# Prayforhanluo/HiCHap_master

Measured on AMD Instinct MI355X. Metric: ICE iterations/sec on 10 kb whole-genome matrix (also nnz*iters/sec), higher is better.
Workload: dtype f64; 1 GPU; hg19-10kb-diploid-wholegenome; n_bins=607282, nnz_upper=4998527599, resolution_bp=10000, parallelism=single GPU, entries_stored=9997055198, slots_u32=160483740, slots_u16=3332512024, payload_bytes=14837255808, tiles=88993, units=88985, hbm_bytes_matrix=15785038153

## Files before the change

### hichap_master_amd/_lib.py

```python
from __future__ import annotations

import ctypes as C
import os

_HERE = os.path.dirname(os.path.abspath(__file__))
LIB_PATH = os.environ.get("HH_LIB") or os.path.join(_HERE, "libhichap_hip.so")

HH_OK = 0


class HipLibraryError(RuntimeError):

    def __init__(self, code, msg):
        super().__init__(f"[hh rc={code}] {msg}")
        self.code = code


class MatrixInfo(C.Structure):
    _fields_ = [(n, C.c_int64) for n in (
        "n_bins", "row_lo", "row_hi", "nnz_upper", "n_entries", "n_slots", "n_tiles",
        "n_units", "n_wide", "device_bytes", "n_slots_narrow", "payload_bytes")] + [
        (n, C.c_int32) for n in ("n_chroms", "ignore_diags", "cis_only", "device", "band_w", "n_units_flat")] + [
        ("n_band", C.c_int64), ("payload_bytes_flat", C.c_int64)] + [
        (n, C.c_int32) for n in ("band_w4", "upper")]
# ... 47 lines not shown
    "hh_ice_n_groups": (C.c_int, [P, PI32]),
    "hh_ice_marg_local": (C.c_int, [P, I32, P, P]),
    "hh_ice_set_marg": (C.c_int, [P, P, I32, I64, P, P]),
    "hh_ice_filter_nnz": (C.c_int, [P, P]),
    "hh_ice_filter_count_mad": (C.c_int, [P, P]),
    "hh_ice_update": (C.c_int, [P, P]),
    "hh_ice_active_groups": (C.c_int, [P, PI32, P]),
    "hh_ice_iterations_done": (C.c_int, [P, PI32]),
    "hh_ice_run": (C.c_int, [P, I32, P]),
    "hh_ice_finalize": (C.c_int, [P, P, P, P, P, P, P]),
    "hh_ice_last_sweep_timing": (C.c_int, [P, PF64, PI32, PF64]),
    "hh_ice_swept_bytes": (C.c_int, [P, PI64]),
    "hh_ice_get_bias": (C.c_int, [P, P, P]),
    "hh_ice_set_bias": (C.c_int, [P, P, P]),
    "hh_ice_uband_fallbacks": (C.c_int, [P, PI64, P]),
    "hh_sweep_trace": (C.c_int, [P, I64, PI64]),
    "hh_matrix_stream_probe": (C.c_int, [P, I32, PF64, I32]),
    "hh_comm_unique_id": (C.c_int, [P]),
    "hh_comm_init": (C.c_int, [P, I32, I32, C.POINTER(P)]),
    "hh_comm_free": (C.c_int, [P]),
    "hh_comm_allgather": (C.c_int, [P, I64, P, P, P]),
    "hh_comm_reduce_scatter": (C.c_int, [P, I64, P, P, P]),
    "hh_ice_set_column_exchange": (C.c_int, [P, I32, I32, P, P, P, P, P]),
    "hh_ice_balance_sharded": (C.c_int, [P, C.POINTER(IceOpts), I32, I32, P, P, P, P, P, P, P, P, PF64, P]),
    "hh_ice_balance_cis_local": (C.c_int, [P, C.POINTER(IceOpts), I32, I64, P, P, P, P, P, P, P, PF64, P]),
    "hh_ice_filters_sharded": (C.c_int, [P, I32, P, P, P, P]),
    "hh_ice_run_sharded": (C.c_int, [P, I32, P, P, P, I32, P]),
    "hh_dense_rowstats": (C.c_int, [P, I32, I64, P, P, P, P, I32, P]),
    "hh_dense_symvc": (C.c_int, [P, I32, I64, P, P, F64, F64, P, I32, P]),
    "hh_twostep": (C.c_int, [P, P, P, I64, P, P, P, P, I32, P]),
# ... 143 lines not shown
```

### hichap_master_amd/csrc/build.hip

```cpp
#include <algorithm>
#include <cmath>
#include <numeric>

#include <chrono>
#include <cstdio>

#include "ice_internal.hpp"

namespace hh {

struct PxErr {
    unsigned long long first;
    int code;
};

constexpr int kOccCopies = 64;

template <class Id, class Cnt>
__global__ __launch_bounds__(256) void k_px_check(const Id* __restrict__ b1, const Id* __restrict__ b2,
                                                  const Cnt* __restrict__ cnt, long long nnz, long long n_bins,
                                                  const int32_t* __restrict__ chrom_of, int ignore_diags,
                                                  int cis_only, int32_t* __restrict__ A, int32_t* __restrict__ B,
                                                  uint32_t* __restrict__ kc, unsigned* __restrict__ occ,
                                                  unsigned* __restrict__ big, int occ_max,
// ... 115 lines not shown
    if (q >= n) return;
    const long long i = (long long)(keys[q] & imask);
    keys[q] = (unsigned long long)(uint32_t)A[i] | ((unsigned long long)kc[i] << 32);
}

struct PxRows {
    const int32_t* A;
    const int32_t* B;
    const uint32_t* kc;
    const long long* up_ptr;
    const unsigned long long* lkeys;
    const long long* lo_ptr;
    long long row_lo, nloc;
    int nJ, band_w, band_w4;
    int upper;
    uint16_t* cnt;
    uint16_t* cntn;
    int32_t* row_band;
    long long* row_wide;
    long long* row_upper;
    long long* row_ent;
    double* diag;
    double* row_nnz2;
    double* row_sum2;
    const int32_t* tile_of;
    const long long* tile_ent;
    const uint32_t* tile_rp;
    const long long* tile_entn;
    const uint32_t* tile_rpn;
    uint32_t* pay;
// ... 2 lines not shown
    uint32_t* band4;
    const long long* wide_ptr;
    int32_t* wide_col;
    double* wide_cnt;
};

template <int PASS>
__global__ __launch_bounds__(256) void k_px_rows(PxRows p) {
    const long long w = ((long long)blockIdx.x * blockDim.x + threadIdx.x) >> 6;
    if (w >= p.nloc) return;
    const int lane = threadIdx.x & 63;
    const long long r = p.row_lo + w;
    const long long rb = w / kR;
    const int k = (int)(w % kR);
    const unsigned long long lt = (1ull << lane) - 1ull;
    int curJ = -1;
    long long tw = 0, tn = 0, pos = 0, posn = 0;
    long long nb_lane = 0, sum_lane = 0, ent_wave = 0, wide_wave = 0, upper_wave = 0;
    long long wpos = PASS == 1 ? p.wide_ptr[w] : 0;
    double dg = 0.0;
    auto flush = [&]() {
        if (curJ < 0) return;
        if (PASS == 0) {
            if (lane == 0) {
                p.cnt[w * p.nJ + curJ] = (uint16_t)tw;
                p.cntn[w * p.nJ + curJ] = (uint16_t)tn;
            }
        } else {
            const long long pw = (tw + 3) & ~3LL, pn = (tn + 7) & ~7LL;
            for (long long q = tw + lane; q < pw; q += 64) p.pay[pos - tw + q] = 0u;
            for (long long q = tn + lane; q < pn; q += 64) p.payn[posn - tn + q] = 0u;
        }
    };
    auto chunk = [&](long long col, uint32_t v, bool valid) {
        if (valid && col == r) {
            dg = (double)v;
            valid = false;
        }
        if (valid) sum_lane += v;
        const long long dj = col - r;
        const bool inband = valid && p.band_w > 0 && v <= kBandMaxCnt && dj >= -p.band_w && dj <= p.band_w;
        const bool innib = valid && !inband && in_band4(dj, v, p.band_w, p.band_w4);
        if (inband || innib) {
            if (PASS == 1) {
                if (inband) {
                    p.band[w * band_stride(p.band_w) + band_slot(dj, p.band_w)] = (uint8_t)v;
                } else {
                    const long long nib = w * 2 * band4_stride(p.band_w, p.band_w4) + band4_nibble(dj, p.band_w, p.band_w4);
                    atomicOr(p.band4 + (nib >> 3), v << (4 * (nib & 7)));
                }
            }
            nb_lane += 1;
            valid = false;
        }
        const bool wide = valid && v > kCntMax;
        const unsigned long long mwl = __ballot(wide);
        if (mwl) {
// ... 220 lines not shown
    DBuf<int32_t> rband(std::max<int64_t>(nloc, 1));
    DBuf<long long> rwide(nloc + 1), rupper(std::max<int64_t>(nloc, 1)), rent(std::max<int64_t>(nloc, 1));
    PxRows P{};
    P.A = dA.p;
    P.B = dB.p;
    P.kc = dkc.p;
    P.up_ptr = up_ptr.p;
    P.lkeys = keys.p;
    P.lo_ptr = lo_ptr.p;
    P.row_lo = row_lo;
    P.nloc = nloc;
    P.nJ = nJ;
    P.band_w = W;
    P.band_w4 = W4;
    P.upper = upper_tiles_on(nJ) ? 1 : 0;
    P.cnt = cnt_w.p;
    P.cntn = cnt_n.p;
    P.row_band = rband.p;
    P.row_wide = rwide.p;
    P.row_upper = rupper.p;
    P.row_ent = rent.p;
    P.diag = m->diag.p;
    P.row_nnz2 = m->row_nnz2.p;
    P.row_sum2 = m->row_sum2.p;
    const dim3 rgrid((unsigned)((nloc * 64 + 255) / 256));
    if (nloc) hipLaunchKernelGGL((k_px_rows<0>), rgrid, dim3(256), 0, s, P);
    HIP_CHECK(hipGetLastError());
    phase("pass 0");
    std::vector<uint16_t> hc((size_t)nloc * nJ), hnarrow((size_t)nloc * nJ);
    std::vector<int32_t> hb(nloc);
// ... 98 lines not shown
```

### hichap_master_amd/csrc/ice.hip

```cpp
#include <algorithm>
#include <chrono>
#include <functional>
#include <cmath>
#include <limits>

#include "ice_internal.hpp"

namespace hh {
constexpr int kThreads = 256;

constexpr int kSweepThreads = 512;
constexpr int kSweepWaves = kSweepThreads / 64;
constexpr int kFlatU = 8;
static_assert(kFlatU == kFlatIlvU, "k_sweep_flatw walks the interleaved layout's runs");

__device__ __forceinline__ double lds_b(const double* bl, uint32_t byteoff) {
    return *reinterpret_cast<const double*>(reinterpret_cast<const char*>(bl) + byteoff);
}

__device__ __forceinline__ void tile_dot(const uint4 v, const double* __restrict__ bl, double& a0, double& a1) {
    const uint32_t w[4] = {v.x, v.y, v.z, v.w};
    double x[4];
#pragma unroll
    for (int i = 0; i < 4; ++i) x[i] = lds_b(bl, w[i] & 0xFFFFu);
// ... 1508 lines not shown
    int bytes;
    int nc, ch, bits;
};
struct UbSegs {
    UbSeg s[2];
    int n;
    uint8_t ord[kMaxUbChunks];
};
struct UbArgs {
    long long row_lo, row_hi, halo_lo, nloc, g_lo;
    const uint8_t* act;
    const uint16_t* row_group;
    const double* b;
    double* upart;
    unsigned long long* fallbacks;
};

template <int BITS>
struct UbT;
template <>
struct UbT<8> {
    typedef uint4 V;
    static constexpr int LB = 16;
    static __device__ __forceinline__ V zero() { return make_uint4(0u, 0u, 0u, 0u); }
    static __device__ __forceinline__ V ld(const uint8_t* p) { return ld16(reinterpret_cast<const uint4*>(p)); }
    template <int M>
    static __device__ __forceinline__ V shift(const V prev, const V own) {
        if (M == 0) return own;
        constexpr int B = 128 - 8 * M;
        return band_shift_q<B / 32>(prev, own, B % 32);
    }
// ... 199 lines not shown
            }
        }
        if (lane == 1) {
#pragma unroll
            for (int k = 0; k < 16; ++k) heads[16 * g + k] = FAST ? col[k] * kUbDown : col[k];
        }
#pragma unroll
        for (int k = 0; k < 16; ++k) col[k] = dpp_shl1_d(col[k]);
    }
    if (FAST) {
#pragma unroll
        for (int k = 0; k < 16; ++k) col[k] *= kUbDown;
    }
}

__device__ __forceinline__ void ub_group(const UbSegs& S, long long grp, int chunk, const UbArgs& a, long long n_bins,
                                         int fast, double* __restrict__ cbuf, double* __restrict__ cwin,
                                         double* __restrict__ rowb) {
    int si = 0;
    while (si + 1 < S.n && chunk >= S.s[si + 1].ch) ++si;
    const UbSeg& P = S.s[si];
    const int kc = chunk - P.ch;
    const long long R0 = grp * kUbGroupRows;
    const int wave = __builtin_amdgcn_readfirstlane(threadIdx.x >> 6), lane = threadIdx.x & 63;
    const long long base = P.dlo + (long long)kc * kUbChunk;
    for (int j = threadIdx.x; j < kUbCols - kUbGroupRows; j += kUbThreads) cbuf[kUbGroupRows + j] = 0.0;
    if (threadIdx.x < 16) cwin[kUbWinZero + threadIdx.x] = 0.0;
    const double up = fast ? kUbUp : 1.0;
    int bad = 0;
    for (int j = threadIdx.x; j < kUbCols; j += kUbThreads) {
        const double v = ub_bias(a.b, R0 + base + j, n_bins);
        bad |= !ub_in_range(v);
        cwin[ub_pad(j)] = v * up;
// ... 6 lines not shown
    if (fast) {
        fast = __builtin_amdgcn_readfirstlane(!__syncthreads_or(bad));
        if (!fast) {
            if (threadIdx.x == 0) atomicAdd(a.fallbacks, 1ull);
            for (int j = threadIdx.x; j < kUbCols; j += kUbThreads) cwin[ub_pad(j)] = ub_bias(a.b, R0 + base + j, n_bins);
            for (int j = threadIdx.x; j < kUbGroupRows; j += kUbThreads) rowb[j] = ub_bias(a.b, R0 + j, n_bins);
            __syncthreads();
        }
    } else {
        __syncthreads();
    }
    const long long r0 = R0 + (long long)kUbRows * wave;
    const bool rows_here = r0 < a.row_hi && r0 + kUbRows > a.row_lo;
    const bool cols_here = r0 + base < a.row_hi && r0 + kUbRows + base + kUbChunk > a.row_lo;
    const bool stored = r0 + kUbRows > a.halo_lo && r0 < a.row_hi;
    double col[16];
    double* heads = cbuf + (size_t)kUbRows * wave;
    if ((rows_here || cols_here) && stored) {
        if (P.bits == 8) {
            if (fast)
                ub_walk<8, true>(P, kc, chunk, r0, a, n_bins, heads, col, cwin, rowb);
            else
                ub_walk<8, false>(P, kc, chunk, r0, a, n_bins, heads, col, cwin, rowb);
        } else {
            if (fast)
                ub_walk<4, true>(P, kc, chunk, r0, a, n_bins, heads, col, cwin, rowb);
            else
                ub_walk<4, false>(P, kc, chunk, r0, a, n_bins, heads, col, cwin, rowb);
        }
    } else {
        for (int j = lane; j < kUbRows; j += 64) heads[j] = 0.0;
#pragma unroll
        for (int k = 0; k < 16; ++k) col[k] = 0.0;
// ... 7 lines not shown
        }
    }
    __syncthreads();
    double* __restrict__ base_p = a.upart + (size_t)(kUbArrs * chunk + 1) * a.nloc;
    for (int j = threadIdx.x; j < kUbCols; j += kUbThreads) {
        const long long c = R0 + base + j;
        if (c >= a.row_lo && c < a.row_hi) base_p[(size_t)(j / kUbGroupRows) * a.nloc + (c - a.row_lo)] = cbuf[j];
    }
}

__global__ __launch_bounds__(kUbThreads, 3) __attribute__((amdgpu_num_vgpr(68))) void k_sweep_ubands(UbSegs S, UbArgs a, long long n_bins, int xcd,
                                                                int fast) {
    __shared__ double cbuf[kUbCols];
    __shared__ double cwin[kUbWin];
    __shared__ double rowb[kUbGroupRows];
    long long grp = blockIdx.x;
    int y = blockIdx.y;
    if (xcd) {
        const long long nb = (long long)gridDim.x * gridDim.y, b = blockIdx.x + (long long)blockIdx.y * gridDim.x;
        const long long L = xcd_remap(b, nb);
        y = (int)(L % gridDim.y);
        grp = L / gridDim.y;
    }
    ub_group(S, a.g_lo + grp, S.ord[y], a, n_bins, fast, cbuf, cwin, rowb);
}

__global__ void k_ub_halo(const uint8_t* __restrict__ band, const uint8_t* __restrict__ band4, long long W8,
                          long long W4, long long row_lo, long long row_hi, long long halo_lo,
                          uint8_t* __restrict__ h8, uint8_t* __restrict__ h4) {
    const long long nh = row_lo - halo_lo;
    const long long st8 = band_stride(W8), st4 = band4_stride(W8, W4), sg = band4_seg(W8, W4);
    const long long per = W8 + (W4 > W8 ? sg : 0);
    const long long i = (long long)blockIdx.x * blockDim.x + threadIdx.x;
    if (i >= nh * per) return;
    const long long hr = i / per, j = i % per, c = halo_lo + hr;
    if (j < W8) {
        const long long d = j + 1, r = c + d;
        if (r >= row_lo && r < row_hi) h8[hr * st8 + W8 + d] = band[(r - row_lo) * st8 + (W8 - d)];
    } else {
// ... 481 lines not shown
struct hh_ice {
    hh_matrix* m = nullptr;
    hh_ice_opts o{};
    int64_t n = 0, nloc = 0;
    int32_t G = 1;
    std::vector<int64_t> glo, ghi;
    int32_t n_tiles = 0;
    DBuf<int32_t> tile_lo, tile_hi, tile_group, group_tile_ptr, blk_tile_ptr;
    DBuf<double> bias, marg, part, tile_cnt, tile_sum, tile_sq, g_cnt, g_sum;
    DBuf<unsigned> counter;
    bool stats_fresh = false;
    DBuf<double> bpart;
    int32_t nch = 0;
    int32_t nchu = 0;
    DBuf<double> upart;
    DBuf<unsigned long long> ub_fallbacks;
    DBuf<uint8_t> halo8, halo4;
    int64_t halo_lo = 0, ub_glo = 0, ub_ghi = 0;
    DBuf<uint8_t> active;
    DBuf<double> g_var, g_mean;
    DBuf<int32_t> g_iters;
    DBuf<uint8_t> g_empty;
    DBuf<long long> rank_rows;
    std::vector<int64_t> h_rank_rows;
    DBuf<unsigned long long> colpart, colacc, bmax, bfix;
    DBuf<double> fix;
    double rmax = 1.0;
    bool rmax_global = false;
    int32_t cx_world = 1, cx_rank = 0;
    int64_t cx_maxlen = 0;
// ... 36 lines not shown
static int g_flatw_waves = 11;
static int g_flatw_waves_up = 8;
static int g_flatw_pipe = 3;
static int g_sweep_ablate = 0;
static int g_tiled_pf = 1;
static int g_band_concurrent = 1;
static int g_split_tiles = 1;
static int g_conc_order = 1;
static int64_t g_conc_min_bytes = 8LL << 30;
static int64_t g_conc_ub_min_bytes = 1LL << 30;
static int g_band_rows = 0;
static int g_band_fused = 1;
static int g_band_lpt = 1;
static int g_uband = 1;
static int64_t g_uband_min_bytes = 128LL << 20;
static int g_ub_xcd = 1;
static int g_ub_fast = 1;
static int g_sweep_single = -1;
static int g_iter_events = 1;
static int64_t g_single_max_bytes = 1LL << 30;
static unsigned long long* g_trace = nullptr;
static int64_t g_trace_cap = 0, g_trace_n = 0;

template <int NB, int ABL, bool UP>
static void launch_sweep_up(const hh_matrix* m, const TileDev& T, const uint8_t* act, const double* b, double* part,
                            hipStream_t s, hipStream_t s_tiled, int which) {
    const int n_tiled = (int)(m->n_units - m->n_units_flat), n_flat = (int)m->n_units_flat;
    auto tiled = [&] {
        if (!n_tiled) return;
        HH_KTIME("k_sweep_tiled", s_tiled);
// ... 123 lines not shown
        const long long sg = band4_seg(W8, W4);
        add(m->band4.p + sg, S->halo4.p ? S->halo4.p + sg : nullptr, band4_stride(W8, W4), W8 + 1, sg, W4 - W8, 4);
    }
    HH_REQUIRE(ch <= kMaxUbChunks, "too many upper-band chunks");
    std::vector<std::pair<long long, int>> w;
    for (int k = 0; k < u.n; ++k)
        for (int c = 0; c < u.s[k].nc; ++c) {
            const long long slots = u.s[k].bits == 8 ? W8 + 1 : W4 - W8;
            w.push_back({-std::min<long long>(kUbChunk, slots + 15 - (long long)c * kUbChunk), u.s[k].ch + c});
        }
    std::stable_sort(w.begin(), w.end(), [](const auto& a, const auto& b) { return a.first < b.first; });
    for (int y = 0; y < ch; ++y) u.ord[y] = (uint8_t)w[y].second;
    return ch;
}

static UbArgs ub_args(hh_ice* S) {
    const hh_matrix* m = S->m;
    return UbArgs{m->row_lo, m->row_hi, S->halo_lo, S->nloc, S->ub_glo, S->act(), m->row_group.p, S->bias.p,
                  S->upart.p, S->ub_fallbacks.p};
}

static UbMarg ub_marg(const hh_ice* S) {
    UbMarg u{};
    u.part = S->upart.p;
    u.n = S->nchu;
    if (!S->nchu) return u;
    UbSegs segs;
    ub_segs(S, segs);
    for (int k = 0; k < segs.n; ++k)
        for (int c = 0; c < segs.s[k].nc; ++c) u.base[segs.s[k].ch + c] = segs.s[k].dlo + (long long)c * kUbChunk;
    return u;
}

static void sweep_uband(hh_ice* S, hipStream_t s) {
    UbSegs segs;
    const int ch = ub_segs(S, segs);
    const long long ng = S->ub_ghi - S->ub_glo;
    if (!ch || ng <= 0) return;
    HH_KTIME("k_sweep_ubands", s);
    hipLaunchKernelGGL(k_sweep_ubands, dim3((unsigned)ng, (unsigned)ch), dim3(kUbThreads), 0, s, segs, ub_args(S),
                       (long long)S->m->n_bins, g_ub_xcd, g_ub_fast);
    HIP_CHECK(hipGetLastError());
}

static void sweep_band(hh_ice* S, hipStream_t s) {
    if (S->nchu) {
        if (S->nloc) sweep_uband(S, s);
        return;
    }
    const hh_matrix* m = S->m;
    if (!S->nch || !S->nloc) return;
    BandSegs segs;
    const int ch = band_segs(m, segs);
    const int rows = g_band_rows ? g_band_rows : (((S->nloc + 255) / 256) * ch < 1024 ? 64 : 256);
    const bool abl = g_sweep_ablate == 1;
// ... 284 lines not shown
        } else if (k == "parse_ablate") {
            HH_REQUIRE(value >= 0 && value <= 3, "parse_ablate in [0, 3]");
            g_parse_ablate = (int)value;
        } else if (k == "flatw_waves") {
            HH_REQUIRE(value == 8 || value == 10 || value == 11, "flatw_waves: 8, 10 or 11");
            g_flatw_waves = (int)value;
        } else if (k == "flat_group") {
            HH_REQUIRE(value >= 0 && value <= 256, "flat_group: 0 (auto) .. 256");
            g_flat_group = value;
        } else if (k == "uband") {
            HH_REQUIRE(value >= 0 && value <= 2, "uband: 0 (off), 1 (auto) or 2 (always)");
            g_uband = (int)value;
        } else if (k == "ub_xcd") {
            HH_REQUIRE(value == 0 || value == 1, "ub_xcd: 0 or 1");
            g_ub_xcd = (int)value;
        } else if (k == "ub_fast") {
            HH_REQUIRE(value == 0 || value == 1, "ub_fast: 0 or 1");
            g_ub_fast = (int)value;
        } else if (k == "uband_min_bytes") {
            HH_REQUIRE(value >= 0, "uband_min_bytes >= 0");
            g_uband_min_bytes = value;
        } else if (k == "band_w") {
            HH_REQUIRE(value >= -1 && value <= kBandMaxW && (value <= 0 || value % 16 == 0),
                       "band_w: -1 (auto), 0 (off) or a multiple of 16 <= 16384");
            g_band_w = value;
        } else if (k == "conc_min_bytes") {
            HH_REQUIRE(value >= 0, "conc_min_bytes >= 0");
            g_conc_min_bytes = value;
        } else if (k == "syrk_split") {
            HH_REQUIRE(value >= -1 && value <= 64, "syrk_split in [-1, 64]");
// ... 178 lines not shown
                    S->halo8.alloc((size_t)(nh * band_stride(W8)));
                    S->halo8.zero(s);
                }
                if (W4 > W8) {
                    S->halo4.alloc((size_t)(nh * band4_stride(W8, W4)));
                    S->halo4.zero(s);
                }
                const long long nthr = nh * per;
                hipLaunchKernelGGL(k_ub_halo, dim3((unsigned)((nthr + 255) / 256)), dim3(256), 0, s, m->band.p,
                                   m->band4.p, W8, W4, (long long)m->row_lo, (long long)m->row_hi, S->halo_lo,
                                   S->halo8.p, S->halo4.p);
                HIP_CHECK(hipGetLastError());
            }
            UbSegs segs;
            S->nchu = ub_segs(S.get(), segs);
            S->upart.alloc(std::max<int64_t>((int64_t)kUbArrs * S->nchu * S->nloc, 1));
            S->upart.zero(s);
            S->ub_fallbacks.alloc(1);
            S->ub_fallbacks.zero(s);
            S->nch = 0;
        }
        S->bpart.alloc(std::max<int64_t>((int64_t)S->nch * S->nloc, 1));
        if (m->upper && m->n_cslots > 0) {
            S->colpart.alloc((size_t)m->n_cslots * kW);
            S->colpart.zero(s);
        }
        if (m->upper) {
            S->colacc.alloc((size_t)std::max<int64_t>(S->n, 1));
            S->colacc.zero(s);
            const unsigned long long one[2] = {0x3FF0000000000000ull, 0ull};
// ... 239 lines not shown
}

int hh_ice_uband_fallbacks(const hh_ice* S, int64_t* count, void* stream) {
    return guard([&] {
        HH_REQUIRE(S && count, "null");
        unsigned long long c = 0;
        if (S->nchu) {
            hipStream_t s = as_stream(stream);
            S->ub_fallbacks.download(&c, 1, s);
            HIP_CHECK(hipStreamSynchronize(s));
        }
        *count = (int64_t)c;
    });
}

int hh_ice_swept_bytes(const hh_ice* S, int64_t* bytes) {
    return guard([&] {
        HH_REQUIRE(S && bytes, "null");
        const hh_matrix* m = S->m;
        int64_t b = 4 * m->n_slots + 2 * m->n_slots_narrow + (int64_t)8 * (kR + 1) * m->n_tiles;
        if (S->nchu) {
            const long long W8 = m->band_w, W4 = m->band_w4;
            const long long per = (W8 > 0 ? W8 + 16 : 0) + (W4 > W8 ? band4_seg(W8, W4) : 0);
            b += (int64_t)per * (S->nloc + (m->row_lo - S->halo_lo));
        } else {
            b += (int64_t)m->band.n + (int64_t)m->band4.n;
        }
        *bytes = b;
    });
}

int hh_matrix_stream_probe(const hh_matrix* m, int32_t reps, double* out, int32_t nout) {
    return guard([&] {
        HH_REQUIRE(m && out && nout >= 20 && reps > 0, "stream probe: 20 outputs");
        for (int i = 0; i < nout; ++i) out[i] = 0.0;
        HIP_CHECK(hipSetDevice(m->device));
        hipStream_t s;
        HIP_CHECK(hipStreamCreateWithFlags(&s, hipStreamNonBlocking));
        hipEvent_t e0, e1;
// ... 219 lines not shown
```

### hichap_master_amd/csrc/ice_internal.hpp

```cpp
#pragma once

#include "hh_common.hpp"

namespace hh {

constexpr int kR = 512;
#ifndef HH_KWBITS
#define HH_KWBITS 13
#endif
constexpr int kWBits = HH_KWBITS;
constexpr bool kUpperBuild = HH_KWBITS <= 12;
constexpr int kW = 1 << kWBits;
constexpr uint32_t kColMask = kW - 1;
constexpr uint32_t kCntMax = 65535u;
extern int64_t g_unit_lpt;
extern int64_t g_unit_lpt_lists;
extern int64_t g_tile_cost;
extern int64_t g_unit_entries;
constexpr int64_t kMaxBins = (int64_t)1 << 30;

constexpr uint32_t kNarrowMax = 7;

constexpr int kBandChunk = 2048;
constexpr int kBandMaxW = 16384;
constexpr uint32_t kBandMaxCnt = 255u;
constexpr double kBandDensity = 0.5;
extern int64_t g_band_w;
constexpr uint32_t kBand4MaxCnt = 15u;
extern double g_band4_density;
extern double g_band8_big;
extern int64_t g_band4;
extern int64_t g_upper_tiles;
struct BandWidths {
    int32_t w8 = 0, w4 = 0;
};
BandWidths choose_band_widths(const std::vector<double>& occ, const std::vector<double>& big, int ignore_diags);
__host__ __device__ __forceinline__ int64_t band4_seg(int64_t w8, int64_t w4) { return w4 > w8 ? (w4 - w8) / 2 + 16 : 0; }
__host__ __device__ __forceinline__ int64_t band4_stride(int64_t w8, int64_t w4) { return 2 * band4_seg(w8, w4); }
__host__ __device__ __forceinline__ int64_t band4_nibble(int64_t d, int64_t w8, int64_t w4) {
    return d < 0 ? d + w4 : 2 * band4_seg(w8, w4) + (d - w8 - 1);
}
__host__ __device__ __forceinline__ bool in_band4(int64_t d, uint32_t v, int64_t w8, int64_t w4) {
    const int64_t a = d < 0 ? -d : d;
    return v > 0 && v <= kBand4MaxCnt && a > w8 && a <= w4;
}
__host__ __device__ __forceinline__ int64_t band_slot(int64_t d, int64_t W) { return d + W; }
// ... 122 lines not shown

struct hh_matrix {
    int device = 0;
    int64_t n_bins = 0, row_lo = 0, row_hi = 0;
    int32_t n_chroms = 0, ignore_diags = 1, cis_only = 0;
    std::vector<int64_t> chrom_offsets;
    int64_t nnz_upper = 0;
    int64_t n_entries = 0;
    int64_t n_tiles = 0, n_units = 0, n_part = 0, n_wide = 0, nJ = 0, nrb = 0;
    int64_t n_units_flat = 0;
    int64_t payload_bytes_flat = 0;
    int64_t n_slots = 0;
    int64_t n_slots_narrow = 0;
    int32_t band_w = 0;
    int32_t band_w4 = 0;
    int64_t n_band = 0;
    hh::DBuf<uint8_t> band;
    hh::DBuf<uint8_t> band4;
    hh::DBuf<uint32_t> pay;
    hh::DBuf<uint16_t> payn;
    hh::DBuf<int32_t> tile_J, tile_rb;
    hh::DBuf<long long> tile_ent, tile_entn;
    hh::DBuf<uint32_t> tile_rp, tile_rpn;
    hh::DBuf<int32_t> u_tlo, u_thi, u_rb, u_rlo, u_rhi, u_slot, blk_unit_ptr, blk_tile_ptr, u_order;
    hh::DBuf<uint16_t> u_glo, u_ghi, tile_perm, tile_band;
    hh::DBuf<uint32_t> tile_fw;
    hh::DBuf<int32_t> tile_frec;
    hh::DBuf<uint16_t> frec;
    hh::DBuf<uint8_t> u_whole;
    hh::DBuf<int32_t> fg_ptr, fg_unit;
// ... 69 lines not shown
```

### hichap_master_amd/csrc/matrix.hip

```cpp
#include <algorithm>
#include <atomic>
#include <chrono>
#include <cstdio>
#include <cmath>
#include <numeric>
#include <exception>
#include <mutex>
#include <thread>

#include "ice_internal.hpp"

namespace hh {

static thread_local std::string g_last_error;
int64_t g_unit_entries = 0;
int g_flat_defer = 1;
int64_t g_unit_lpt = 1;
int64_t g_unit_lpt_lists = 1;
int64_t g_flat_group = 0;
int64_t g_flat_cols = -1;
bool flat_cols_on(int32_t nJ) { return g_flat_cols > 0 || (g_flat_cols < 0 && nJ >= 32); }
int64_t g_tile_cost = 32768;
int64_t g_band_w = -1;
int64_t g_flat_max = 64;
int64_t g_build_debug = 0;
int64_t g_host_build = 0;

int64_t g_upper_tiles = -1;
bool upper_tiles_on(int32_t nJ) {
    return kUpperBuild && (g_upper_tiles > 0 || (g_upper_tiles < 0 && flat_cols_on(nJ)));
}
int64_t g_band4 = 1;
double g_band4_density = 0.25;
double g_band8_big = 0.05;

int32_t choose_band_w(const std::vector<double>& occ, int ignore_diags) {
    if (g_band_w >= 0) return (int32_t)std::min<int64_t>(g_band_w, kBandMaxW) & ~15;
    int64_t d = std::max(1, ignore_diags);
    if (d > 1) return 0;
    while (d < (int64_t)occ.size() && occ[d] >= kBandDensity) ++d;
    return (int32_t)((d - 1) & ~15LL);
}

BandWidths choose_band_widths(const std::vector<double>& occ, const std::vector<double>& big, int ignore_diags) {
    BandWidths bw;
    bw.w8 = bw.w4 = choose_band_w(occ, ignore_diags);
    if (g_band_w >= 0 || !g_band4 || std::max(1, ignore_diags) > 1) return bw;
// ... 653 lines not shown
            for (int64_t i = 0; i < nnz; ++i) {
                int64_t a, b;
                uint32_t c;
                if (!keep(i, a, b, c) || a == b || b - a > kBandMaxW + 1) continue;
                occ[b - a] += 1.0;
                if (c > kBand4MaxCnt) big[b - a] += 1.0;
            }
            for (int64_t d = 1; d < (int64_t)occ.size(); ++d) {
                big[d] = occ[d] > 0 ? big[d] / occ[d] : 0.0;
                occ[d] = d < n_bins ? occ[d] / (double)(n_bins - d) : 0.0;
            }
            const BandWidths bw = choose_band_widths(occ, big, ignore_diags);
            W = bw.w8;
            W4 = bw.w4;
        }
        auto in_band = [&](int64_t r_glob, int64_t col, uint32_t v) {
            const int64_t d = col - r_glob;
            return W > 0 && v <= kBandMaxCnt && d != 0 && d >= -W && d <= W;
        };
        auto in_nib = [&](int64_t r_glob, int64_t col, uint32_t v) { return in_band4(col - r_glob, v, W, W4); };
        std::vector<int32_t> cols(deg[nloc]);
        std::vector<uint32_t> vals(deg[nloc]);
        {
            std::vector<int64_t> pos(deg.begin(), deg.end() - 1);
            for (int64_t i = 0; i < nnz; ++i) {
                int64_t a, b;
                uint32_t c;
                if (!keep(i, a, b, c) || a == b) continue;
                if (a >= row_lo && a < row_hi) { cols[pos[a - row_lo]] = (int32_t)b; vals[pos[a - row_lo]++] = c; }
                if (b >= row_lo && b < row_hi) { cols[pos[b - row_lo]] = (int32_t)a; vals[pos[b - row_lo]++] = c; }
            }
        }
        std::vector<std::pair<int32_t, uint32_t>> tmp;
        for (int64_t r = 0; r < nloc; ++r) {
            const int64_t lo = deg[r], hi = deg[r + 1];
// ... 218 lines not shown
```

### hichap_master_amd/csrc/synth.hip

```cpp
#include <cmath>
#include <numeric>

#include "ice_internal.hpp"

namespace hh {

struct SynthDev {
    long long n;
    int n_chroms;
    int nJ;
    const int* chrom_lo;
    const float* vis;
    const signed char* sgn;
    const short* chrom;
    float A, decay, comp, trans;
    int ignore_diags, cis_only;
    unsigned long long seed;
    int band_w;
    int band_w4;
    int ordered;
    int upper;
};

__global__ void k_synth_bins(SynthDev p, float vis_sigma, float gap_frac, int comp_block,
                             float* vis, signed char* sgn) {
    const long long i = (long long)blockIdx.x * blockDim.x + threadIdx.x;
    if (i >= p.n) return;
    const int c = p.chrom[i];
    const long long local = i - p.chrom_lo[c];
    const uint64_t h = mix64(p.seed ^ mix64(0xB1A5ull + (uint64_t)i));
    const float u1 = fmaxf(u01(h), 1e-7f), u2 = u01(mix64(h));
    const float z = sqrtf(-2.f * logf(u1)) * cosf(6.2831853f * u2);
    const bool gap = u01(mix64(h ^ 0x5151ull)) < gap_frac;
    vis[i] = gap ? 0.f : expf(vis_sigma * z);
    const uint64_t hb = mix64(p.seed ^ mix64(0xC0FFEEull + ((uint64_t)c << 32) + (uint64_t)(local / comp_block)));
    sgn[i] = (hb & 1) ? 1 : -1;
// ... 53 lines not shown
    uint16_t* payn;
    uint8_t* band;
    uint32_t* band4;
    int32_t* row_band;
};

template <int PASS>
__global__ __launch_bounds__(256) void k_synth_rows(SynthDev p, long long row_lo, long long nrows, SynthOut o) {
    const long long w = ((long long)blockIdx.x * blockDim.x + threadIdx.x) >> 6;
    if (w >= nrows) return;
    const int lane = threadIdx.x & 63;
    const long long r = row_lo + w;
    const int c = p.chrom[r];
    const long long jlo = p.cis_only ? p.chrom_lo[c] : 0;
    const long long jhi = p.cis_only ? p.chrom_lo[c + 1] : p.n;
    const long long rb = w / kR;
    const int k = (int)(w % kR);
    const unsigned long long lt_mask = (lane == 0) ? 0ull : (~0ull >> (64 - lane));
    long long upper = 0, nnz = 0, work = 0, sum_lane = 0, nb_lane = 0, nbu_lane = 0, nd_lane = 0;
    const int Jr = (int)(r >> kWBits);
    int curJ = -1;
    long long tw = 0, tn = 0;
    long long pos = 0, posn = 0;
    auto flush = [&]() {
        if (curJ < 0) return;
        if (PASS == 0) {
            if (lane == 0 && o.cnt) {
                o.cnt[w * p.nJ + curJ] = (uint16_t)tw;
                o.cntn[w * p.nJ + curJ] = (uint16_t)tn;
            }
        } else {
            const long long pw = (tw + 3) & ~3LL, pn = (tn + 7) & ~7LL;
            for (long long q = tw + lane; q < pw; q += 64) o.pay[pos - tw + q] = 0u;
            for (long long q = tn + lane; q < pn; q += 64) o.payn[posn - tn + q] = 0u;
        }
        work += ((tw + 3) & ~3LL) + ((tn + 7) & ~7LL) / 2;
    };
    for (long long j0 = jlo & ~63LL; j0 < jhi; j0 += 64) {
        const long long j = j0 + lane;
        const int J = (int)(j0 >> kWBits);
        uint32_t kc = 0;
        if (j >= jlo && j < jhi && j != r) kc = synth_count(p, r, j);
        const long long dj = j - r;
        const bool inband = kc > 0 && p.band_w > 0 && kc <= kBandMaxCnt && dj >= -p.band_w && dj <= p.band_w;
        const bool innib = !inband && in_band4(dj, kc, p.band_w, p.band_w4);
        if (inband || innib) {
            if (PASS == 1) {
                if (inband) {
                    o.band[w * band_stride(p.band_w) + band_slot(dj, p.band_w)] = (uint8_t)kc;
                } else {
                    const long long nib = w * 2 * band4_stride(p.band_w, p.band_w4) + band4_nibble(dj, p.band_w, p.band_w4);
                    atomicOr(o.band4 + (nib >> 3), kc << (4 * (nib & 7)));
                }
            }
            nb_lane += 1;
            nbu_lane += dj > 0 ? 1 : 0;
            sum_lane += kc;
            kc = 0;
        }
        if (p.upper && kc > 0 && J < Jr) {
// ... 91 lines not shown
    d.n = n;
    d.n_chroms = p->n_chroms;
    d.nJ = (int)((n + kW - 1) / kW);
    d.chrom_lo = h.chrom_lo.p;
    d.vis = h.vis.p;
    d.sgn = h.sgn.p;
    d.chrom = h.chrom.p;
    d.A = (float)p->A;
    d.decay = (float)p->decay;
    d.comp = (float)p->comp_strength;
    d.trans = (float)p->trans_density;
    d.ignore_diags = p->ignore_diags;
    d.cis_only = p->cis_only ? 1 : 0;
    d.seed = p->seed;
    d.upper = upper_tiles_on(d.nJ) ? 1 : 0;
    {
        const BandWidths bw = synth_band_w(p, h.offsets);
        d.band_w = bw.w8;
        d.band_w4 = bw.w4;
    }
    hipLaunchKernelGGL(k_synth_bins, dim3((unsigned)((n + 255) / 256)), dim3(256), 0, s, d,
                       (float)p->vis_sigma, (float)p->gap_frac, p->comp_block, h.vis.p, h.sgn.p);
    HIP_CHECK(hipGetLastError());
}

inline dim3 row_grid(int64_t nrows) { return dim3((unsigned)((nrows * 64 + 255) / 256)); }

BandWidths synth_band_w(const hh_synth_params* p, const std::vector<int64_t>& offsets) {
    const int S = 2048;
    std::vector<double> x(S);
// ... 153 lines not shown
        std::vector<int32_t> hb(nloc);
        rband.download(hb.data(), nloc, s);
        HIP_CHECK(hipStreamSynchronize(s));
        cnt.release();
        cntn.release();
        std::vector<uint16_t> bg = bin_groups(*m);
        std::vector<uint16_t> rgroup(bg.begin() + row_lo, bg.begin() + row_hi);
        TilePlan P = plan_tiles(hc.data(), hn.data(), nloc, nJ, rgroup, row_lo, h.dev.upper != 0);
        upload_plan(P, *m, s);
        m->row_group = to_device(rgroup, s);
        DBuf<int32_t> tof = to_device(P.tile_of, s);
        m->pay.alloc(P.n_entries_padded);
        m->payn.alloc(P.n_narrow_padded);
        m->band_w = h.dev.band_w;
        m->band_w4 = h.dev.band_w4;
        m->band.alloc((size_t)nloc * band_stride(m->band_w));
        m->band.zero(s);
        m->band4.alloc((size_t)nloc * band4_stride(m->band_w, m->band_w4));
        m->band4.zero(s);
        {
            SynthOut o{};
            o.band = m->band.p;
            o.band4 = reinterpret_cast<uint32_t*>(m->band4.p);
            o.tile_of = tof.p;
            o.tile_ent = m->tile_ent.p;
            o.tile_rp = m->tile_rp.p;
            o.tile_entn = m->tile_entn.p;
            o.tile_rpn = m->tile_rpn.p;
            o.pay = m->pay.p;
            o.payn = m->payn.p;
// ... 84 lines not shown
```

### hichap_master_amd/ice.py

```python
from __future__ import annotations

import ctypes as C
from dataclasses import asdict, dataclass

import numpy as np

from . import _lib
from ._lib import IceOpts, MatrixInfo, SynthParams, call, ptr


@dataclass
class IceOptions:
    ignore_diags: int = 1
    cis_only: bool = False
    mad_max: int = 5
    min_nnz: int = 10
    min_count: float = 0
    tol: float = 1e-5
    max_iters: int = 200
    rescale_marginals: bool = True
    check_every: int = 8

    def c_opts(self) -> IceOpts:
        return IceOpts(int(self.mad_max), int(self.min_nnz), float(self.min_count), float(self.tol),
# ... 256 lines not shown
        b = np.empty(int(self.m.info()["n_bins"]))
        call("hh_ice_get_bias", self._h, ptr(b), stream)
        return b

    def set_bias(self, b, stream=None):
        b = np.ascontiguousarray(b, dtype=np.float64)
        if b.shape != (int(self.m.info()["n_bins"]),):
            raise ValueError("set_bias: one bias per bin")
        call("hh_ice_set_bias", self._h, ptr(b), stream)

    def uband_fallbacks(self, stream=None) -> int:
        n = C.c_int64(0)
        call("hh_ice_uband_fallbacks", self._h, C.byref(n), stream)
        return n.value

    def finalize(self, stream=None):
        n = int(self.m.info()["n_bins"])
        G = self.n_groups
        w = np.empty(n)
        scale, var = np.empty(G), np.empty(G)
        iters, conv = np.empty(G, np.int32), np.empty(G, np.int32)
        call("hh_ice_finalize", self._h, ptr(w), ptr(scale), ptr(var), ptr(iters), ptr(conv), stream)
        return w, _stats(self.opts, scale, var, iters, conv, self.m.info()["cis_only"])

    def close(self):
        if self._h:
            call("hh_ice_free", self._h)
            self._h = None

    def __del__(self):
# ... 9 lines not shown
```

### include/hichap_hip.h

```cpp
#ifndef HICHAP_HIP_H
#define HICHAP_HIP_H

#include <stdint.h>

#ifdef __cplusplus
extern "C" {
#endif

#define HH_OK 0
#define HH_ERR_ARG -1
#define HH_ERR_HIP -2
#define HH_ERR_OOM -3
#define HH_ERR_STATE -4

const char* hh_last_error(void);
int hh_version(void);
int hh_device_count(int32_t* n);
int hh_set_device(int32_t device);
int hh_synchronize(void* stream);
int hh_device_copy(void* dst, const void* src, int64_t bytes, void* stream);
int hh_tune(const char* key, int64_t value);
int hh_sweep_trace(uint64_t* out, int64_t cap, int64_t* n);
int hh_ktime_enable(int32_t on);
int hh_ktime_query(const char* name, double* total_ms, int64_t* calls);
// ... 88 lines not shown
                    const int64_t* rank_rows, void* stream);
int hh_ice_filter_nnz(hh_ice* s, void* stream);
int hh_ice_filter_count_mad(hh_ice* s, void* stream);
int hh_ice_update(hh_ice* s, void* stream);
int hh_ice_active_groups(hh_ice* s, int32_t* n_active, void* stream);
int hh_ice_iterations_done(const hh_ice* s, int32_t* iters);
int hh_ice_run(hh_ice* s, int32_t n, void* stream);
int hh_ice_finalize(hh_ice* s, double* weights, double* scale, double* var, int32_t* iters,
                    int32_t* converged, void* stream);
int hh_ice_last_sweep_timing(const hh_ice* s, double* sweep_ms_total, int32_t* sweep_launches,
                             double* iter_ms_total);
int hh_ice_swept_bytes(const hh_ice* s, int64_t* bytes);
int hh_ice_get_bias(const hh_ice* s, double* bias, void* stream);
int hh_ice_set_bias(hh_ice* s, const double* bias, void* stream);
int hh_ice_uband_fallbacks(const hh_ice* s, int64_t* count, void* stream);

typedef int (*hh_allgather_fn)(const double* send, int64_t count, double* recv, void* user, void* stream);
typedef struct hh_comm hh_comm;
int hh_comm_unique_id(uint8_t* id128);
int hh_comm_init(const uint8_t* id128, int32_t world, int32_t rank, hh_comm** out);
int hh_comm_free(hh_comm* c);
int hh_comm_allgather(const double* send, int64_t count, double* recv, void* comm, void* stream);
typedef int (*hh_reduce_fn)(const int64_t* send, int64_t count, int64_t* recv, void* user, void* stream);
int hh_comm_reduce_scatter(const int64_t* send, int64_t count, int64_t* recv, void* comm, void* stream);
int hh_ice_set_column_exchange(hh_ice* s, int32_t world, int32_t rank, const int64_t* rank_rows, hh_reduce_fn reduce,
                               void* reduce_user, hh_allgather_fn allgather, void* allgather_user);
int hh_ice_balance_sharded(hh_matrix* m, const hh_ice_opts* o, int32_t world, int32_t rank, const int64_t* rank_rows,
                           hh_allgather_fn allgather, void* user, double* weights, double* scale, double* var,
                           int32_t* iters, int32_t* converged, double* sweep_seconds, void* stream);
int hh_ice_balance_cis_local(hh_matrix* m, const hh_ice_opts* o, int32_t world, int64_t max_local_bins,
// ... 177 lines not shown
```

Baseline: 354.0 ICE iterations/s.

## Restrict diagonal band storage to cis entries and skip dead uband waves

Band and nibble-band storage now only takes entries whose column lies on the same chromosome as the row. Trans near-diagonal entries at chromosome boundaries go to the regular tile payload instead. A host-side plan builds a compact task list of (group, chunk, dead-wave mask) for the uband sweep. Fully dead workgroups are never launched and dead waves skip their walk, so the kernel avoids streaming band bytes past chromosome ends. This adds a task-table load per block and a host planning pass at setup, and it changes the build layout of the band.

```diff
diff --git a/hichap_master_amd/_lib.py b/hichap_master_amd/_lib.py
--- a/hichap_master_amd/_lib.py
+++ b/hichap_master_amd/_lib.py
@@ -85,6 +85,7 @@
     "hh_ice_get_bias": (C.c_int, [P, P, P]),
     "hh_ice_set_bias": (C.c_int, [P, P, P]),
     "hh_ice_uband_fallbacks": (C.c_int, [P, PI64, P]),
+    "hh_ice_uband_skipped": (C.c_int, [P, PI64, PI64]),
     "hh_sweep_trace": (C.c_int, [P, I64, PI64]),
     "hh_matrix_stream_probe": (C.c_int, [P, I32, PF64, I32]),
     "hh_comm_unique_id": (C.c_int, [P]),
diff --git a/hichap_master_amd/csrc/build.hip b/hichap_master_amd/csrc/build.hip
--- a/hichap_master_amd/csrc/build.hip
+++ b/hichap_master_amd/csrc/build.hip
@@ -153,6 +153,8 @@
     long long row_lo, nloc;
     int nJ, band_w, band_w4;
     int upper;
+    const int32_t* chrom_of;
+    const long long* chrom_lo;
     uint16_t* cnt;
     uint16_t* cntn;
     int32_t* row_band;
@@ -185,6 +187,12 @@
     const long long rb = w / kR;
     const int k = (int)(w % kR);
     const unsigned long long lt = (1ull << lane) - 1ull;
+    long long cis_lo = 0, cis_hi = kMaxBins;
+    if (p.chrom_of) {
+        const int c = p.chrom_of[r];
+        cis_lo = p.chrom_lo[c];
+        cis_hi = p.chrom_lo[c + 1];
+    }
     int curJ = -1;
     long long tw = 0, tn = 0, pos = 0, posn = 0;
     long long nb_lane = 0, sum_lane = 0, ent_wave = 0, wide_wave = 0, upper_wave = 0;
@@ -210,8 +218,9 @@
         }
         if (valid) sum_lane += v;
         const long long dj = col - r;
-        const bool inband = valid && p.band_w > 0 && v <= kBandMaxCnt && dj >= -p.band_w && dj <= p.band_w;
-        const bool innib = valid && !inband && in_band4(dj, v, p.band_w, p.band_w4);
+        const bool cis = col >= cis_lo && col < cis_hi;
+        const bool inband = valid && cis && p.band_w > 0 && v <= kBandMaxCnt && dj >= -p.band_w && dj <= p.band_w;
+        const bool innib = valid && cis && !inband && in_band4(dj, v, p.band_w, p.band_w4);
         if (inband || innib) {
             if (PASS == 1) {
                 if (inband) {
@@ -462,6 +471,10 @@
     P.band_w = W;
     P.band_w4 = W4;
     P.upper = upper_tiles_on(nJ) ? 1 : 0;
+    m->band_cis = g_band_cis ? 1 : 0;
+    DBuf<long long> dclo = to_device(std::vector<long long>(chrom_offsets, chrom_offsets + n_chroms + 1), s);
+    P.chrom_of = m->band_cis ? dch.p : nullptr;
+    P.chrom_lo = dclo.p;
     P.cnt = cnt_w.p;
     P.cntn = cnt_n.p;
     P.row_band = rband.p;
diff --git a/hichap_master_amd/csrc/ice.hip b/hichap_master_amd/csrc/ice.hip
--- a/hichap_master_amd/csrc/ice.hip
+++ b/hichap_master_amd/csrc/ice.hip
@@ -1546,7 +1546,15 @@
     const double* b;
     double* upart;
     unsigned long long* fallbacks;
+    const uint32_t* tasks;
 };
+
+constexpr int kUbTaskGrpBits = 22, kUbTaskChunkBits = 6;
+static_assert((kMaxBins >> 9) <= (1ll << kUbTaskGrpBits) && kUbGroupRows == 512, "workgroup index bits of a task word");
+static_assert(kMaxUbChunks <= (1 << kUbTaskChunkBits) && kUbWaves == 32 - kUbTaskGrpBits - kUbTaskChunkBits, "task word");
+__host__ __device__ __forceinline__ uint32_t ub_task(long long grp, int chunk, unsigned dead) {
+    return (uint32_t)grp | ((uint32_t)chunk << kUbTaskGrpBits) | (dead << (kUbTaskGrpBits + kUbTaskChunkBits));
+}
 
 template <int BITS>
 struct UbT;
@@ -1776,9 +1784,9 @@
     }
 }
 
-__device__ __forceinline__ void ub_group(const UbSegs& S, long long grp, int chunk, const UbArgs& a, long long n_bins,
-                                         int fast, double* __restrict__ cbuf, double* __restrict__ cwin,
-                                         double* __restrict__ rowb) {
+__device__ __forceinline__ void ub_group(const UbSegs& S, long long grp, int chunk, unsigned dead, const UbArgs& a,
+                                         long long n_bins, int fast, double* __restrict__ cbuf,
+                                         double* __restrict__ cwin, double* __restrict__ rowb) {
     int si = 0;
     while (si + 1 < S.n && chunk >= S.s[si + 1].ch) ++si;
     const UbSeg& P = S.s[si];
@@ -1815,9 +1823,10 @@
     const bool rows_here = r0 < a.row_hi && r0 + kUbRows > a.row_lo;
     const bool cols_here = r0 + base < a.row_hi && r0 + kUbRows + base + kUbChunk > a.row_lo;
     const bool stored = r0 + kUbRows > a.halo_lo && r0 < a.row_hi;
+    const bool live = !((dead >> wave) & 1u);
     double col[16];
     double* heads = cbuf + (size_t)kUbRows * wave;
-    if ((rows_here || cols_here) && stored) {
+    if ((rows_here || cols_here) && stored && live) {
         if (P.bits == 8) {
             if (fast)
                 ub_walk<8, true>(P, kc, chunk, r0, a, n_bins, heads, col, cwin, rowb);
@@ -1855,15 +1864,11 @@
     __shared__ double cbuf[kUbCols];
     __shared__ double cwin[kUbWin];
     __shared__ double rowb[kUbGroupRows];
-    long long grp = blockIdx.x;
-    int y = blockIdx.y;
-    if (xcd) {
-        const long long nb = (long long)gridDim.x * gridDim.y, b = blockIdx.x + (long long)blockIdx.y * gridDim.x;
-        const long long L = xcd_remap(b, nb);
-        y = (int)(L % gridDim.y);
-        grp = L / gridDim.y;
-    }
-    ub_group(S, a.g_lo + grp, S.ord[y], a, n_bins, fast, cbuf, cwin, rowb);
+    const long long L = xcd ? xcd_remap(blockIdx.x, gridDim.x) : (long long)blockIdx.x;
+    const uint32_t t = a.tasks[L];
+    ub_group(S, a.g_lo + (long long)(t & ((1u << kUbTaskGrpBits) - 1u)),
+             (int)((t >> kUbTaskGrpBits) & ((1u << kUbTaskChunkBits) - 1u)), t >> (kUbTaskGrpBits + kUbTaskChunkBits), a,
+             n_bins, fast, cbuf, cwin, rowb);
 }
 
 __global__ void k_ub_halo(const uint8_t* __restrict__ band, const uint8_t* __restrict__ band4, long long W8,
@@ -2375,6 +2380,8 @@
     int32_t nch = 0;
     int32_t nchu = 0;
     DBuf<double> upart;
+    DBuf<uint32_t> ub_tasks[2];
+    int64_t ub_ntasks[2] = {0, 0}, ub_bytes[2] = {0, 0}, ub_waves_all = 0, ub_waves_dead = 0;
     DBuf<unsigned long long> ub_fallbacks;
     DBuf<uint8_t> halo8, halo4;
     int64_t halo_lo = 0, ub_glo = 0, ub_ghi = 0;
@@ -2441,6 +2448,7 @@
 static int g_band_lpt = 1;
 static int g_uband = 1;
 static int64_t g_uband_min_bytes = 128LL << 20;
+static int g_ub_skip = 1;
 static int g_ub_xcd = 1;
 static int g_ub_fast = 1;
 static int g_sweep_single = -1;
@@ -2594,10 +2602,74 @@
     return ch;
 }
 
+static void ub_plan(hh_ice* S, const UbSegs& u, int ch, hipStream_t s) {
+    const hh_matrix* m = S->m;
+    const long long n = m->n_bins, ng = S->ub_ghi - S->ub_glo;
+    const long long nblk = std::max<long long>(ng, 0) * kUbWaves, blk0 = S->ub_glo * kUbWaves;
+    const long long never = std::numeric_limits<long long>::max();
+    const bool cis = m->band_cis != 0;
+    std::vector<long long> room(nblk, cis ? 0 : never), room15(nblk, cis ? 0 : never);
+    if (cis)
+        for (int c = 0; c < m->n_chroms; ++c) {
+            const long long end = m->chrom_offsets[c + 1];
+            const long long lo = std::max<long long>(m->chrom_offsets[c], blk0 * kUbRows);
+            const long long hi = std::min<long long>(end, (blk0 + nblk) * kUbRows);
+            for (long long r = lo; r < hi; ++r) {
+                const long long b = r / kUbRows - blk0;
+                room[b] = std::max(room[b], end - r);
+                room15[b] = std::max(room15[b], end - r + (r & 15));
+            }
+        }
+    std::vector<long long> cbytes(ch, 0);
+    for (int k = 0; k < u.n; ++k) {
+        const UbSeg& P = u.s[k];
+        const long long full = (long long)kUbChunk * P.bits / 8;
+        for (int c = 0; c < P.nc; ++c)
+            cbytes[P.ch + c] = c + 1 < P.nc ? std::min<long long>(full, std::max<long long>(P.bytes - c * full, 0))
+                                            : std::max<long long>(P.bytes - c * full, 0);
+    }
+    std::vector<uint32_t> tasks[2];
+    S->ub_bytes[0] = S->ub_bytes[1] = 0;
+    S->ub_waves_all = S->ub_waves_dead = 0;
+    for (long long g = 0; g < ng; ++g)
+        for (int y = 0; y < ch; ++y) {
+            const int chunk = u.ord[y];
+            int si = 0;
+            while (si + 1 < u.n && chunk >= u.s[si + 1].ch) ++si;
+            const int kc = chunk - u.s[si].ch;
+            const long long base = u.s[si].dlo + (long long)kc * kUbChunk;
+            unsigned dead = 0;
+            for (int w = 0; w < kUbWaves; ++w) {
+                const long long b = g * kUbWaves + w, r0 = (blk0 + b) * kUbRows;
+                const bool d = (kc > 0 ? room15[b] : room[b]) <= base;
+                if (d) dead |= 1u << w;
+                if (r0 < n) {
+                    ++S->ub_waves_all;
+                    S->ub_waves_dead += d ? 1 : 0;
+                }
+                const bool rows_here = r0 < m->row_hi && r0 + kUbRows > m->row_lo;
+                const bool cols_here = r0 + base < m->row_hi && r0 + kUbRows + base + kUbChunk > m->row_lo;
+                const bool stored = r0 + kUbRows > S->halo_lo && r0 < m->row_hi;
+                if ((rows_here || cols_here) && stored) {
+                    const long long by = (std::min<long long>(m->row_hi, r0 + kUbRows) - r0) * cbytes[chunk];
+                    S->ub_bytes[0] += by;
+                    if (!d) S->ub_bytes[1] += by;
+                }
+            }
+            tasks[0].push_back(ub_task(g, chunk, 0u));
+            if (dead != (1u << kUbWaves) - 1u) tasks[1].push_back(ub_task(g, chunk, dead));
+        }
+    for (int q = 0; q < 2; ++q) {
+        S->ub_ntasks[q] = (int64_t)tasks[q].size();
+        if (tasks[q].empty()) tasks[q].push_back(0u);
+        S->ub_tasks[q] = to_device(tasks[q], s);
+    }
+}
+
 static UbArgs ub_args(hh_ice* S) {
     const hh_matrix* m = S->m;
     return UbArgs{m->row_lo, m->row_hi, S->halo_lo, S->nloc, S->ub_glo, S->act(), m->row_group.p, S->bias.p,
-                  S->upart.p, S->ub_fallbacks.p};
+                  S->upart.p, S->ub_fallbacks.p, S->ub_tasks[g_ub_skip ? 1 : 0].p};
 }
 
 static UbMarg ub_marg(const hh_ice* S) {
@@ -2615,10 +2687,10 @@
 static void sweep_uband(hh_ice* S, hipStream_t s) {
     UbSegs segs;
     const int ch = ub_segs(S, segs);
-    const long long ng = S->ub_ghi - S->ub_glo;
-    if (!ch || ng <= 0) return;
+    const long long nt = S->ub_ntasks[g_ub_skip ? 1 : 0];
+    if (!ch || nt <= 0) return;
     HH_KTIME("k_sweep_ubands", s);
-    hipLaunchKernelGGL(k_sweep_ubands, dim3((unsigned)ng, (unsigned)ch), dim3(kUbThreads), 0, s, segs, ub_args(S),
+    hipLaunchKernelGGL(k_sweep_ubands, dim3((unsigned)nt), dim3(kUbThreads), 0, s, segs, ub_args(S),
                        (long long)S->m->n_bins, g_ub_xcd, g_ub_fast);
     HIP_CHECK(hipGetLastError());
 }
@@ -2933,6 +3005,12 @@
         } else if (k == "ub_xcd") {
             HH_REQUIRE(value == 0 || value == 1, "ub_xcd: 0 or 1");
             g_ub_xcd = (int)value;
+        } else if (k == "ub_skip") {
+            HH_REQUIRE(value == 0 || value == 1, "ub_skip: 0 or 1");
+            g_ub_skip = (int)value;
+        } else if (k == "band_cis") {
+            HH_REQUIRE(value == 0 || value == 1, "band_cis: 0 or 1");
+            g_band_cis = value;
         } else if (k == "ub_fast") {
             HH_REQUIRE(value == 0 || value == 1, "ub_fast: 0 or 1");
             g_ub_fast = (int)value;
@@ -3141,6 +3219,7 @@
             }
             UbSegs segs;
             S->nchu = ub_segs(S.get(), segs);
+            ub_plan(S.get(), segs, S->nchu, s);
             S->upart.alloc(std::max<int64_t>((int64_t)kUbArrs * S->nchu * S->nloc, 1));
             S->upart.zero(s);
             S->ub_fallbacks.alloc(1);
@@ -3410,15 +3489,21 @@
     });
 }
 
+int hh_ice_uband_skipped(const hh_ice* S, int64_t* dead_waves, int64_t* all_waves) {
+    return guard([&] {
+        HH_REQUIRE(S && dead_waves && all_waves, "null");
+        *dead_waves = S->nchu ? S->ub_waves_dead : 0;
+        *all_waves = S->nchu ? S->ub_waves_all : 0;
+    });
+}
+
 int hh_ice_swept_bytes(const hh_ice* S, int64_t* bytes) {
     return guard([&] {
         HH_REQUIRE(S && bytes, "null");
         const hh_matrix* m = S->m;
         int64_t b = 4 * m->n_slots + 2 * m->n_slots_narrow + (int64_t)8 * (kR + 1) * m->n_tiles;
         if (S->nchu) {
-            const long long W8 = m->band_w, W4 = m->band_w4;
-            const long long per = (W8 > 0 ? W8 + 16 : 0) + (W4 > W8 ? band4_seg(W8, W4) : 0);
-            b += (int64_t)per * (S->nloc + (m->row_lo - S->halo_lo));
+            b += S->ub_bytes[g_ub_skip ? 1 : 0];
         } else {
             b += (int64_t)m->band.n + (int64_t)m->band4.n;
         }
diff --git a/hichap_master_amd/csrc/ice_internal.hpp b/hichap_master_amd/csrc/ice_internal.hpp
--- a/hichap_master_amd/csrc/ice_internal.hpp
+++ b/hichap_master_amd/csrc/ice_internal.hpp
@@ -30,6 +30,7 @@
 extern double g_band4_density;
 extern double g_band8_big;
 extern int64_t g_band4;
+extern int64_t g_band_cis;
 extern int64_t g_upper_tiles;
 struct BandWidths {
     int32_t w8 = 0, w4 = 0;
@@ -182,6 +183,7 @@
     int64_t n_slots_narrow = 0;
     int32_t band_w = 0;
     int32_t band_w4 = 0;
+    int32_t band_cis = 0;
     int64_t n_band = 0;
     hh::DBuf<uint8_t> band;
     hh::DBuf<uint8_t> band4;
diff --git a/hichap_master_amd/csrc/matrix.hip b/hichap_master_amd/csrc/matrix.hip
--- a/hichap_master_amd/csrc/matrix.hip
+++ b/hichap_master_amd/csrc/matrix.hip
@@ -31,6 +31,7 @@
     return kUpperBuild && (g_upper_tiles > 0 || (g_upper_tiles < 0 && flat_cols_on(nJ)));
 }
 int64_t g_band4 = 1;
+int64_t g_band_cis = 1;
 double g_band4_density = 0.25;
 double g_band8_big = 0.05;
 
@@ -714,11 +715,15 @@
             W = bw.w8;
             W4 = bw.w4;
         }
+        m->band_cis = g_band_cis ? 1 : 0;
+        auto cis_ok = [&](int64_t r_glob, int64_t col) { return !m->band_cis || chrom_of[r_glob] == chrom_of[col]; };
         auto in_band = [&](int64_t r_glob, int64_t col, uint32_t v) {
             const int64_t d = col - r_glob;
-            return W > 0 && v <= kBandMaxCnt && d != 0 && d >= -W && d <= W;
+            return W > 0 && v <= kBandMaxCnt && d != 0 && d >= -W && d <= W && cis_ok(r_glob, col);
         };
-        auto in_nib = [&](int64_t r_glob, int64_t col, uint32_t v) { return in_band4(col - r_glob, v, W, W4); };
+        auto in_nib = [&](int64_t r_glob, int64_t col, uint32_t v) {
+            return in_band4(col - r_glob, v, W, W4) && cis_ok(r_glob, col);
+        };
         std::vector<int32_t> cols(deg[nloc]);
         std::vector<uint32_t> vals(deg[nloc]);
         {
diff --git a/hichap_master_amd/csrc/synth.hip b/hichap_master_amd/csrc/synth.hip
--- a/hichap_master_amd/csrc/synth.hip
+++ b/hichap_master_amd/csrc/synth.hip
@@ -20,6 +20,7 @@
     int band_w4;
     int ordered;
     int upper;
+    int band_cis;
 };
 
 __global__ void k_synth_bins(SynthDev p, float vis_sigma, float gap_frac, int comp_block,
@@ -103,6 +104,7 @@
     const int c = p.chrom[r];
     const long long jlo = p.cis_only ? p.chrom_lo[c] : 0;
     const long long jhi = p.cis_only ? p.chrom_lo[c + 1] : p.n;
+    const long long cis_lo = p.chrom_lo[c], cis_hi = p.chrom_lo[c + 1];
     const long long rb = w / kR;
     const int k = (int)(w % kR);
     const unsigned long long lt_mask = (lane == 0) ? 0ull : (~0ull >> (64 - lane));
@@ -131,8 +133,9 @@
         uint32_t kc = 0;
         if (j >= jlo && j < jhi && j != r) kc = synth_count(p, r, j);
         const long long dj = j - r;
-        const bool inband = kc > 0 && p.band_w > 0 && kc <= kBandMaxCnt && dj >= -p.band_w && dj <= p.band_w;
-        const bool innib = !inband && in_band4(dj, kc, p.band_w, p.band_w4);
+        const bool cis = !p.band_cis || (j >= cis_lo && j < cis_hi);
+        const bool inband = cis && kc > 0 && p.band_w > 0 && kc <= kBandMaxCnt && dj >= -p.band_w && dj <= p.band_w;
+        const bool innib = cis && !inband && in_band4(dj, kc, p.band_w, p.band_w4);
         if (inband || innib) {
             if (PASS == 1) {
                 if (inband) {
@@ -254,6 +257,7 @@
     d.cis_only = p->cis_only ? 1 : 0;
     d.seed = p->seed;
     d.upper = upper_tiles_on(d.nJ) ? 1 : 0;
+    d.band_cis = g_band_cis ? 1 : 0;
     {
         const BandWidths bw = synth_band_w(p, h.offsets);
         d.band_w = bw.w8;
@@ -437,6 +441,7 @@
         m->payn.alloc(P.n_narrow_padded);
         m->band_w = h.dev.band_w;
         m->band_w4 = h.dev.band_w4;
+        m->band_cis = h.dev.band_cis;
         m->band.alloc((size_t)nloc * band_stride(m->band_w));
         m->band.zero(s);
         m->band4.alloc((size_t)nloc * band4_stride(m->band_w, m->band_w4));
diff --git a/hichap_master_amd/ice.py b/hichap_master_amd/ice.py
--- a/hichap_master_amd/ice.py
+++ b/hichap_master_amd/ice.py
@@ -294,6 +294,11 @@
         call("hh_ice_uband_fallbacks", self._h, C.byref(n), stream)
         return n.value
 
+    def uband_skipped(self):
+        dead, tot = C.c_int64(0), C.c_int64(0)
+        call("hh_ice_uband_skipped", self._h, C.byref(dead), C.byref(tot))
+        return dead.value, tot.value
+
     def finalize(self, stream=None):
         n = int(self.m.info()["n_bins"])
         G = self.n_groups
diff --git a/include/hichap_hip.h b/include/hichap_hip.h
--- a/include/hichap_hip.h
+++ b/include/hichap_hip.h
@@ -126,6 +126,7 @@
 int hh_ice_get_bias(const hh_ice* s, double* bias, void* stream);
 int hh_ice_set_bias(hh_ice* s, const double* bias, void* stream);
 int hh_ice_uband_fallbacks(const hh_ice* s, int64_t* count, void* stream);
+int hh_ice_uband_skipped(const hh_ice* s, int64_t* dead_waves, int64_t* all_waves);
 
 typedef int (*hh_allgather_fn)(const double* send, int64_t count, double* recv, void* user, void* stream);
 typedef struct hh_comm hh_comm;
```

New measurement: 385.9 ICE iterations/s (median of 6 runs). 9.0% higher.
